# reinterpretcat/qwen3-rs

Hardware: NVIDIA B200
Metric: decode_tokens_per_s (higher is better)
Workload: dtype int8 weights x int8 activations, int32 group dots, f32 accumulate

## Files before the change

### qwen3_rs_b200/csrc/q3_engine.cu

```cuda
#include "../../include/qwen3_cuda.h"
#include "q3_kernels.cuh"
#include "q3_mega.cuh"
#include "q3_prefill.cuh"
#include "q3_sampler.cuh"
#include <cudaTypedefs.h>

#include <cuda_runtime.h>
#include <fcntl.h>
#include <math.h>
#include <stdarg.h>
#include <stdio.h>
#include <stdlib.h>
#include <string.h>
#include <sys/mman.h>
#include <sys/stat.h>
#include <unistd.h>

#include <string>
#include <vector>

using namespace q3;

static thread_local char g_err[1024] = "";
static int fail(int code, const char *fmt, ...) {
// ... 593 lines not shown
    CK(cudaFuncSetAttribute(h->mega_fn, cudaFuncAttributeMaxDynamicSharedMemorySize, (int)h->mega_smem));
    int occ = 0;
    CK(cudaOccupancyMaxActiveBlocksPerMultiprocessor(&occ, h->mega_fn, MEGA_THREADS, h->mega_smem));
    if (occ < 1) { h->mega_why = "megakernel does not fit on an SM"; return 0; }
    h->mega_ok = true;
    return 0;
}

static int launch_mega(q3_handle *h, int l0, int l1, bool from_embed, bool run_head, bool feedback, bool gather) {
    MegaArgs a = h->margs;
    a.layer0 = l0; a.layer1 = l1; a.from_embed = from_embed; a.run_head = run_head; a.feedback = feedback;
    a.gather_logits = h->tp_size > 1 ? (h->logits_root >= 0 ? (1 << h->logits_root) : (gather ? (1 << h->tp_size) - 1 : 0)) : 0;
    a.bar_base = h->bar_base;
    a.xbar_base = h->xbar_base;
    if (h->poisoned) return fail(Q3_ECOMM, "tensor-parallel handle is unusable after a timed-out wait (ranks may have diverged): destroy and re-create every rank");
    const int nbar = run_head ? 1 : 0;
    const int nx = h->tp_size > 1 ? nbar : 0;
    a.ll_base = (unsigned)(h->ll_count % 0xFFFFFFFFull);
    h->ll_count += (unsigned long long)MEGA_EDGES * (unsigned)(l1 - l0 + 1);
    void *params[] = {&a};
    CK(cudaLaunchCooperativeKernel(h->mega_fn, dim3(h->num_sms), dim3(MEGA_THREADS), params, h->mega_smem, h->stream));
    h->bar_base += (unsigned long long)(nbar - nx) * h->num_sms;
    h->xbar_base += (unsigned long long)nx * h->tp_size * h->num_sms;
    return 0;
}

static int check_tok_pos(const q3_handle *h, int token, int pos);
static int finish_call(q3_handle *h) {
    const bool mega = h->d_status && h->decode_path == 1;
    if (mega) CK(cudaMemcpyAsync(h->h_small + 16, h->d_status, 4, cudaMemcpyDeviceToHost, h->stream));
    CK(cudaStreamSynchronize(h->stream));
    if (!mega) return 0;
    const int code = h->h_small[16];
    if (code) {
        cudaMemset(h->d_status, 0, 64);
        if (h->tp_size > 1) {
            h->poisoned = true;
        } else {
            h->bar_base = 0;
            h->xbar_base = 0;
            cudaMemset(h->d_bar, 0, 64);
            cudaMemset(h->d_flags, 0, 64 * 4);
            if (h->att_cnt) cudaMemset(h->att_cnt, 0, (size_t)h->cfg.n_layers * h->n_kv_l * 4);
        }
        return fail(Q3_ECUDA, "persistent decode kernel: a wait timed out (status %d: 1 grid barrier, 2 stage ring, 3 cross-GPU barrier, 4 producer order, "
                              "6-10 flagged exchange: 6 o/down rows, 7 attention output, 8 SwiGLU outputs, 9 qkv rows, 10 TP partials; 11 prefill cross-GPU barrier)%s", code,
                    h->tp_size > 1 ? "; tensor-parallel handle poisoned" : "");
    }
    return 0;
}
extern "C" int q3_debug_profile(q3_handle *h, int token, int pos, unsigned long long *out, size_t out_words, int *n_rows_out,
                                int *n_events_out) {
    if (!h) return fail(Q3_EINVAL, "null argument");
    if (n_rows_out) *n_rows_out = 3 * h->num_sms;
    if (n_events_out) *n_events_out = MEGA_PROF_EVENTS;
    if (!out) return out_words == 0 ? Q3_OK : fail(Q3_EINVAL, "null argument");
    if (!h->mega_ok) return fail(Q3_EUNSUPPORTED, "persistent decode kernel unavailable: %s", h->mega_why.c_str());
    if (out_words < (size_t)3 * h->num_sms * MEGA_PROF_EVENTS)
        return fail(Q3_EINVAL, "profile buffer too small: %zu words, need %zu", out_words, (size_t)3 * h->num_sms * MEGA_PROF_EVENTS);
    if (int rc0 = check_tok_pos(h, token, pos)) return rc0;
    CK(cudaSetDevice(h->device));
    h->h_small[0] = token; h->h_small[1] = pos; h->h_small[2] = 0; h->h_small[3] = 0;
    CK(cudaMemcpyAsync(h->d_tokpos, h->h_small, 16, cudaMemcpyHostToDevice, h->stream));
    unsigned long long *d = nullptr;
    size_t bytes = (size_t)3 * h->num_sms * MEGA_PROF_EVENTS * 8;
    CK(cudaMalloc((void **)&d, bytes));
    CK(cudaMemsetAsync(d, 0, bytes, h->stream));
    h->margs.prof = d;
    int rc = launch_mega(h, 0, h->cfg.n_layers, true, true, false, false);
    h->margs.prof = nullptr;
    if (!rc) {
        cudaError_t e = cudaMemcpyAsync(out, d, bytes, cudaMemcpyDeviceToHost, h->stream);
        rc = e == cudaSuccess ? finish_call(h) : fail(Q3_ECUDA, "profile copy failed: %s", cudaGetErrorString(e));
    }
    cudaFree(d);
    return rc;
}
extern "C" int q3_num_sms(const q3_handle *h) { return h ? h->num_sms : 0; }
extern "C" int q3_debug_set_epoch(q3_handle *h, unsigned long long exchanges_issued) {
    if (!h) return fail(Q3_EINVAL, "null handle");
    h->ll_count = exchanges_issued;
    return Q3_OK;
}

static inline bool use_mega(const q3_handle *h) { return h->decode_path == 1 && h->mega_ok && !h->exact; }
static int tp_ready(const q3_handle *h) {
    if (h->tp_size > 1 && !h->tp_connected) return fail(Q3_ECOMM, "tensor-parallel handle used before q3_tp_connect");
    if (h->tp_size > 1 && !use_mega(h)) return fail(Q3_EUNSUPPORTED, "under tensor parallelism only the persistent fast path is available");
    return 0;
}

enum StepOut {
    STEP_LOGITS,
    STEP_ARGMAX,
    STEP_FEEDBACK,
};
static int launch_decode_step(q3_handle *h, StepOut out, bool gather = false) {
    if (use_mega(h)) return launch_mega(h, 0, h->cfg.n_layers, true, true, out == STEP_FEEDBACK, gather);
    CK(cudaGraphLaunch(out == STEP_FEEDBACK ? h->g_greedy[h->exact] : h->g_fwd[h->exact], h->stream));
    if (out == STEP_ARGMAX) launch_argmax(h, false, h->stream);
    return 0;
}
static int launch_head_only(q3_handle *h, bool gather) {
    if (use_mega(h)) return launch_mega(h, 0, 0, false, true, false, gather);
    launch_head(h, h->stream);
    return 0;
}

static PFN_cuTensorMapEncodeTiled_v12000 get_encode_fn() {
    static PFN_cuTensorMapEncodeTiled_v12000 fn = nullptr;
    if (!fn) {
        void *p = nullptr;
        cudaDriverEntryPointQueryResult qres;
        if (cudaGetDriverEntryPoint("cuTensorMapEncodeTiled", &p, cudaEnableDefault, &qres) == cudaSuccess && qres == cudaDriverEntryPointSuccess)
            fn = (PFN_cuTensorMapEncodeTiled_v12000)p;
    }
    return fn;
}
// ... 1292 lines not shown
```

### qwen3_rs_b200/csrc/q3_mega.cuh

```cuda
#pragma once
#include <cuda.h>

#include "q3_kernels.cuh"

namespace q3 {

#ifndef MEGA_GW_
#define MEGA_GW_ 8
#endif
constexpr int MEGA_GW = MEGA_GW_;
constexpr int MEGA_BATCH = 4 * MEGA_GW;
constexpr int MEGA_GROUPS = 2;
constexpr int MEGA_NCW = MEGA_GW * MEGA_GROUPS;
constexpr int MEGA_CTHREADS = MEGA_NCW * 32;
constexpr int MEGA_THREADS = MEGA_CTHREADS + 32 * MEGA_GROUPS;
#ifndef MEGA_NSTAGE_
#define MEGA_NSTAGE_ 4
#endif
constexpr int MEGA_NSTAGE = MEGA_NSTAGE_;
constexpr int MEGA_MAX_KT = 4096;
constexpr int MEGA_SCRATCH = 40960;
constexpr int MEGA_MAX_TP = 8;
constexpr int MEGA_MAX_SPLITS = ATTN_MAX_SPLITS;
constexpr int MEGA_EDGES = 6;

enum { PH_QKV = 0, PH_O = 1, PH_GU = 2, PH_DN = 3, PH_HEAD = 4 };

struct MegaGemv {
    const uint8_t *base;
    long long layer_stride;
    int units;
    int K, n_kt, KT, G;
    int tile_bytes;
};

constexpr int MEGA_KV_ROWS = 32;

struct MegaArgs {
    alignas(64) CUtensorMap map_k;
    alignas(64) CUtensorMap map_v;
    int dim, n_layers, n_heads_l, n_kv_l, AH_l, KV_l, H_l, vocab_l, vocab_row0, seq_len;
    int tp_rank, tp_size;
    MegaGemv g[5];
    const float *rms_att, *rms_ffn, *q_ln, *k_ln, *rms_final;
    const int8_t *embed_q;
    const float *embed_s;
    const float *rope;
    float *kc, *vc;
    float *x;
    unsigned long long *zq;
    unsigned long long *za;
    unsigned long long *zh;
    unsigned long long *zr[2];
    unsigned long long *part[2][MEGA_MAX_TP];
    float *attn_part;
    unsigned *att_cnt;
    float *logits[MEGA_MAX_TP];
    unsigned long long *best[MEGA_MAX_TP];
    unsigned long long *bar;
    unsigned long long bar_base;
    unsigned long long *xbar[MEGA_MAX_TP];
    unsigned long long xbar_base;
    int *tokpos, *history;
    int *status;
    int layer0, layer1, from_embed, run_head, feedback, gather_logits;
    unsigned ll_base;
    unsigned long long *prof;
};
constexpr int MEGA_PROF_EVENTS = 4096;
struct Prof {
    unsigned long long *row;
    int ev;
};
// ... 75 lines not shown
    unsigned long long x;
    asm volatile("ld.relaxed.sys.global.b64 %0, [%1];" : "=l"(x) : "l"(p) : "memory");
    return x;
}
__device__ __forceinline__ bool ll_ok(unsigned long long w, unsigned epoch) { return (unsigned)(w >> 32) == epoch; }
__device__ __noinline__ bool ll_give_up(const MegaArgs &a, unsigned &spins, int code) {
    if ((++spins & 255u) == 0) {
        if (*(volatile int *)a.status) return true;
        if (spins > (1u << 20)) {
            atomicExch(a.status, code);
            return true;
        }
    }
    return false;
}
__device__ __forceinline__ float4 ll_poll4(const MegaArgs &a, const unsigned long long *p, unsigned epoch, int code) {
    unsigned long long w0, w1, w2, w3;
    unsigned spins = 0;
    while (true) {
        ll_load2(p, w0, w1);
        ll_load2(p + 2, w2, w3);
        if (ll_ok(w0, epoch) && ll_ok(w1, epoch) && ll_ok(w2, epoch) && ll_ok(w3, epoch)) break;
        if (ll_give_up(a, spins, code)) break;
    }
    return make_float4(__uint_as_float((unsigned)w0), __uint_as_float((unsigned)w1), __uint_as_float((unsigned)w2), __uint_as_float((unsigned)w3));
}

__device__ __host__ __forceinline__ void cta_share(int units, int nctas, int c, int &start, int &count) {
    int base = units / nctas, rem = units % nctas;
    count = base + (c < rem ? 1 : 0);
    start = c * base + (c < rem ? c : rem);
}

template <int GS>
__global__ void __launch_bounds__(256) k_build_stream(const int8_t *__restrict__ src_q, const float *__restrict__ src_s,
                                                      uint8_t *dst, int units, int K, int n_kt, int nctas, int pair) {
    constexpr int CPG = GS / 16;
    const int u = blockIdx.x, kt = blockIdx.y;
    const int KT = K / n_kt, G = KT / GS, tile_bytes = KT + ((4 * G + 15) & ~15);
    const int base = units / nctas, rem = units % nctas;
    int c, j;
    if (u < rem * (base + 1)) {
        c = u / (base + 1);
        j = u % (base + 1);
    } else {
        c = rem + (u - rem * (base + 1)) / base;
        j = (u - rem * (base + 1)) % base;
    }
    int start, n_c;
    cta_share(units, nctas, c, start, n_c);
    for (int half = 0; half < (pair ? 2 : 1); half++) {
        long long tile_index;
        size_t src_row;
        if (pair) {
            int blk = j / MEGA_GW, w = j % MEGA_GW, np = n_c - MEGA_GW * blk;
            if (np > MEGA_GW) np = MEGA_GW;
            tile_index = (long long)start * 2 + 2 * MEGA_GW * blk + half * np + w;
            src_row = (size_t)2 * u + half;
        } else {
            int b = j / MEGA_BATCH, jb = j % MEGA_BATCH, nb = n_c - MEGA_BATCH * b;
            if (nb > MEGA_BATCH) nb = MEGA_BATCH;
            tile_index = ((long long)start + MEGA_BATCH * b) * n_kt + (long long)kt * nb + jb;
            src_row = (size_t)u;
        }
        uint8_t *tile = dst + tile_index * tile_bytes;
        const int8_t *srow = src_q + src_row * K + (size_t)kt * KT;
        for (int ch = threadIdx.x; ch < KT / 16; ch += blockDim.x) {
            int g = ch / CPG, p = ch % CPG, b = g / 32, l = g % 32;
            int ngb = G - 32 * b;
            if (ngb > 32) ngb = 32;
            int dpos = b * 32 * CPG + p * ngb + l;
            reinterpret_cast<int4 *>(tile)[dpos] = reinterpret_cast<const int4 *>(srow)[ch];
        }
        const float *ss = src_s + src_row * (K / GS) + (size_t)kt * G;
        for (int g = threadIdx.x; g < G; g += blockDim.x) reinterpret_cast<float *>(tile + KT)[g] = ss[g];
    }
}

__device__ __forceinline__ int4 lds128(uint32_t saddr) {
    int4 r;
    asm volatile("ld.shared.v4.b32 {%0,%1,%2,%3}, [%4];" : "=r"(r.x), "=r"(r.y), "=r"(r.z), "=r"(r.w) : "r"(saddr));
    return r;
}
__device__ __forceinline__ float lds_f32(uint32_t saddr) {
    float r;
    asm volatile("ld.shared.f32 %0, [%1];" : "=f"(r) : "r"(saddr));
    return r;
}
template <int GS>
struct XRegs {
    static constexpr int CPG = GS / 16;
    static constexpr int NBLK = MEGA_MAX_KT / (32 * GS);
    int4 x[NBLK][CPG];
    float s[NBLK];
};

template <int GS>
__device__ __forceinline__ int xq_offset(int i4, int KT, int G) {
    int r = i4 * 4, off = 0;
    while (r >= KT) {
        r -= KT;
        off += KT;
    }
    const int g = r / GS, b = g >> 5, l = g & 31;
    int ngb = G - 32 * b;
    ngb = ngb > 32 ? 32 : ngb;
    const int p = (r % GS) >> 4;
    return off + b * 32 * GS + (p * ngb + l) * 16 + (r & 15);
}
template <int GS>
__device__ __forceinline__ void xq_store(uint8_t *sxq, int i4, uint32_t packed, int KT, int G) {
    *reinterpret_cast<uint32_t *>(sxq + xq_offset<GS>(i4, KT, G)) = packed;
}
template <int GS>
__device__ __forceinline__ void load_x(XRegs<GS> &xr, const uint8_t *sxq, const float *sxs, int kt, int KT, int G, int lane) {
    const uint32_t base = smem_u32(sxq) + kt * KT + lane * 16;
#pragma unroll
    for (int b = 0; b < XRegs<GS>::NBLK; b++) {
        int ngb = G - 32 * b;
        ngb = ngb > 32 ? 32 : ngb;
        const bool ok = lane < ngb;
        if (ngb < 1) ngb = 1;
        xr.s[b] = ok ? sxs[kt * G + b * 32 + lane] : 0.0f;
#pragma unroll
        for (int p = 0; p < XRegs<GS>::CPG; p++)
            xr.x[b][p] = ok ? lds128(base + b * 32 * GS + p * ngb * 16) : make_int4(0, 0, 0, 0);
    }
}

template <int GS, bool FULL>
__device__ __forceinline__ float tile_dot(uint32_t tile, const XRegs<GS> &xr, int KT, int G, int lane) {
    constexpr int CPG = XRegs<GS>::CPG;
    constexpr int NBLK = XRegs<GS>::NBLK;
    int4 w[NBLK][CPG];
    float ws[NBLK];
#pragma unroll
    for (int b = 0; b < NBLK; b++) {
        int ngb = FULL ? 32 : (G - 32 * b > 32 ? 32 : G - 32 * b);
        const bool on = FULL ? (32 * b < G) : (lane < ngb);
        if (!FULL && ngb < 1) ngb = 1;
        const uint32_t base = tile + b * 32 * GS + lane * 16;
#pragma unroll
        for (int p = 0; p < CPG; p++) w[b][p] = on ? lds128(base + p * ngb * 16) : make_int4(0, 0, 0, 0);
        ws[b] = on ? lds_f32(tile + KT + (b * 32 + lane) * 4) : 0.0f;
    }
    float acc = 0.0f;
#pragma unroll
    for (int b = 0; b < NBLK; b++) {
        int d0 = 0, d1 = 0;
#pragma unroll
        for (int p = 0; p < CPG; p += 2) {
            d0 = dot16(w[b][p], xr.x[b][p], d0);
            d1 = dot16(w[b][p + 1], xr.x[b][p + 1], d1);
        }
        acc = __fadd_rn(acc, __fmul_rn(__fmul_rn((float)(d0 + d1), ws[b]), xr.s[b]));
    }
    return warp_sum(acc);
}

constexpr int MEGA_MAXV = (MEGA_MAX_KT + 4 * MEGA_CTHREADS - 1) / (4 * MEGA_CTHREADS);

template <int GS>
__device__ __noinline__ void prologue_norm(const MegaArgs &a, const float *w, int src, const unsigned long long *zone, unsigned epoch,
                                           uint8_t *sxq, float *sxs, float *sred, float *sx, int KT, int G, Prof &pr) {
    const int tid = threadIdx.x, lane = tid & 31, warp = tid >> 5;
    const int n4 = a.dim >> 2;
    constexpr int MAXV = MEGA_MAXV;
    float4 v[MAXV], wv[MAXV];
    float ss = 0.0f;
#pragma unroll
    for (int k = 0; k < MAXV; k++) {
        const int i4 = tid + k * MEGA_CTHREADS;
        wv[k] = (i4 < n4) ? __ldg(reinterpret_cast<const float4 *>(w) + i4) : make_float4(0.f, 0.f, 0.f, 0.f);
    }
#pragma unroll
    for (int k = 0; k < MAXV; k++) {
        const int i4 = tid + k * MEGA_CTHREADS;
        v[k] = make_float4(0.f, 0.f, 0.f, 0.f);
        if (i4 < n4) {
            if (src == 0) {
                size_t base = (size_t)a.tokpos[0] * a.dim + (size_t)i4 * 4;
                char4 e = *reinterpret_cast<const char4 *>(a.embed_q + base);
                float sc = a.embed_s[base / GS];
                v[k] = make_float4((float)e.x * sc, (float)e.y * sc, (float)e.z * sc, (float)e.w * sc);
            } else if (src == 1) {
                v[k] = ldcg_f4(a.x + (size_t)i4 * 4);
            } else {
                v[k] = reinterpret_cast<const float4 *>(sx)[i4];
            }
        }
    }
    if (zone) {
        unsigned long long ww[MAXV][4];
        unsigned spins = 0;
        while (true) {
            bool ok = true;
#pragma unroll
            for (int k = 0; k < MAXV; k++) {
                const int i4 = tid + k * MEGA_CTHREADS;
                if (i4 < n4) {
                    ll_load2(zone + (size_t)i4 * 4, ww[k][0], ww[k][1]);
                    ll_load2(zone + (size_t)i4 * 4 + 2, ww[k][2], ww[k][3]);
                    ok = ok && ll_ok(ww[k][0], epoch) && ll_ok(ww[k][1], epoch) && ll_ok(ww[k][2], epoch) && ll_ok(ww[k][3], epoch);
                }
            }
            if (ok || ll_give_up(a, spins, 6)) break;
        }
#pragma unroll
// ... 474 lines not shown
                asm volatile("ld.acquire.gpu.global.u64 %0, [%1];" : "=l"(v) : "l"(a.bar) : "memory");
                if (v >= bs.target) break;
                if ((++spins & 1023u) == 0) {
                    if (*st) break;
                    if (clock64() - t0 > 4000000000LL) {
                        atomicExch(a.status, 1);
                        break;
                    }
                }
            }
        }
    }
    if (x) bs.xtarget += (unsigned long long)a.tp_size * gridDim.x;
    else bs.target += gridDim.x;
    prof_mark(pr, 41);
    csync();
}

struct PhaseGeom {
    const uint8_t *seg;
    int start, count;
};
struct MegaShared {
    int start[5], count[5];
    long long seg_off[5], seg_len[5];
    unsigned long long *part[2][MEGA_MAX_TP];
    float *logits[MEGA_MAX_TP];
    unsigned long long *best[MEGA_MAX_TP];
};
__device__ __forceinline__ PhaseGeom phase_geom(const MegaArgs &a, const MegaShared &sh, int ph, int layer) {
    PhaseGeom pg;
    pg.start = sh.start[ph];
    pg.count = sh.count[ph];
    pg.seg = a.g[ph].base + (long long)layer * a.g[ph].layer_stride + sh.seg_off[ph];
    return pg;
}

template <int GS, int KVMUL>
__global__ void __launch_bounds__(MEGA_THREADS, 1) k_mega_decode(const __grid_constant__ MegaArgs a) {
    extern __shared__ __align__(1024) uint8_t mega_smem[];
    uint8_t *smem = mega_smem;
    const int slot_bytes = MEGA_GW * (MEGA_MAX_KT + 4 * (MEGA_MAX_KT / GS));
    uint8_t *ring = smem;
    uint8_t *scratch = smem + MEGA_NSTAGE * slot_bytes;
    uint8_t *sxq = scratch;
    float *sxs = reinterpret_cast<float *>(scratch + 16384);
    float *sred = reinterpret_cast<float *>(scratch + 16384 + 2048);
    uint64_t *full = reinterpret_cast<uint64_t *>(scratch + MEGA_SCRATCH);
    uint64_t *empty = full + MEGA_GROUPS * MEGA_NSTAGE;
    MegaShared &sh = *reinterpret_cast<MegaShared *>(scratch + MEGA_SCRATCH + 192);
    static_assert(192 + sizeof(MegaShared) <= 1024, "MegaShared outgrew its slot");
    float *sx = reinterpret_cast<float *>(scratch + MEGA_SCRATCH + 1024);
    volatile unsigned *issued = reinterpret_cast<volatile unsigned *>(scratch + MEGA_SCRATCH + 128);
    const int tid = threadIdx.x, lane = tid & 31, warp = tid >> 5;

    if (tid == 0) {
        for (int s = 0; s < MEGA_NSTAGE; s++) {
            mbar_init(&full[s], 1);
            mbar_init(&full[MEGA_NSTAGE + s], 1);
            mbar_init(&empty[s], MEGA_GW);
            issued[s] = 0;
        }
        asm volatile("fence.mbarrier_init.release.cluster;" ::: "memory");
#pragma unroll 1
        for (int ph = 0; ph < 5; ph++) {
            int st, cn;
            cta_share(a.g[ph].units, gridDim.x, blockIdx.x, st, cn);
            const long long per_unit = (long long)(ph == PH_GU ? 2 : 1) * a.g[ph].n_kt * a.g[ph].tile_bytes;
            sh.start[ph] = st;
            sh.count[ph] = cn;
            sh.seg_off[ph] = st * per_unit;
            sh.seg_len[ph] = cn * per_unit;
        }
    }
    if (tid < MEGA_MAX_TP) {
        sh.part[0][tid] = a.part[0][tid];
        sh.part[1][tid] = a.part[1][tid];
        sh.logits[tid] = a.logits[tid];
        sh.best[tid] = a.best[tid];
    }
    __syncthreads();

    const int L0 = a.layer0, L1 = a.layer1;

    if (warp >= MEGA_NCW) {
        if (lane != 0) return;
        const int pw = warp - MEGA_NCW;
        uint64_t policy;
        asm volatile("createpolicy.fractional.L2::evict_first.b64 %0, 1.0;" : "=l"(policy));
        unsigned it = 0;
        Prof pr;
        pr.row = (a.prof && pw == 0) ? a.prof + (size_t)(gridDim.x + blockIdx.x) * MEGA_PROF_EVENTS : nullptr;
        pr.ev = 0;
        auto push = [&](const uint8_t *src, int nr, int tile_bytes, int owner) {
            if (owner != pw) {
                it++;
                return;
            }
            const int slot = it % MEGA_NSTAGE;
            const uint32_t bytes = (uint32_t)nr * tile_bytes;
            {
                const unsigned use = it / MEGA_NSTAGE;
                long long t0 = clock64();
                while (issued[slot] != use) {
                    if (clock64() - t0 > 4000000000LL) { atomicExch(a.status, 4); break; }
                }
            }
            mbar_wait(&empty[slot], ((it / MEGA_NSTAGE) & 1) ^ 1, a.status);
            uint64_t *fb = &full[owner * MEGA_NSTAGE + slot];
            mbar_expect_tx(fb, bytes);
            bulk_g2s(ring + (size_t)slot * slot_bytes, src, bytes, fb, policy);
            __threadfence_block();
            issued[slot] = it / MEGA_NSTAGE + 1;
            prof_mark(pr, 64 + slot);
            it++;
        };
        const int ppos = a.tokpos[1];
        const int pns = mega_nsplit(ppos, a.n_kv_l, gridDim.x);
        const bool has_item = (int)blockIdx.x < a.n_kv_l * pns;
        const int pkvh = blockIdx.x % a.n_kv_l, psplit = blockIdx.x / a.n_kv_l;
        const int pper = (ppos + 1 + pns - 1) / pns;
        const int pt0 = psplit * pper, pt1 = pt0 + pper < ppos + 1 ? pt0 + pper : ppos + 1;
        auto kvpush = [&](int layer) {
            if (!has_item) return;
            for (int t = pt0, si = 0; t < pt1; t += MEGA_KV_ROWS, si++) {
                const int owner = si & 1;
                if (owner != pw) {
                    it++;
                    continue;
                }
                const int slot = it % MEGA_NSTAGE;
                {
                    const unsigned use = it / MEGA_NSTAGE;
                    long long tw = clock64();
                    while (issued[slot] != use) {
                        if (clock64() - tw > 4000000000LL) { atomicExch(a.status, 4); break; }
                    }
                }
                mbar_wait(&empty[slot], ((it / MEGA_NSTAGE) & 1) ^ 1, a.status);
                uint64_t *fb = &full[owner * MEGA_NSTAGE + slot];
                uint8_t *dst = ring + (size_t)slot * slot_bytes;
                mbar_expect_tx(fb, 2 * MEGA_KV_ROWS * HEAD_DIM * 4);
                tma_load_2d(dst, &a.map_k, pkvh * HEAD_DIM, layer * a.seq_len + t, fb);
                tma_load_2d(dst + MEGA_KV_ROWS * HEAD_DIM * 4, &a.map_v, pkvh * HEAD_DIM, layer * a.seq_len + t, fb);
                __threadfence_block();
                issued[slot] = it / MEGA_NSTAGE + 1;
                prof_mark(pr, 64 + slot);
                it++;
            }
        };
        auto plain = [&](int ph, int layer) {
            const MegaGemv &g = a.g[ph];
            PhaseGeom pg = phase_geom(a, sh, ph, layer);
            const uint8_t *src = pg.seg;
            for (int b0 = 0; b0 < pg.count; b0 += MEGA_BATCH) {
                int nb = pg.count - b0 < MEGA_BATCH ? pg.count - b0 : MEGA_BATCH;
                for (int kt = 0; kt < g.n_kt; kt++)
                    for (int s = 0, si = 0; s < nb; s += MEGA_GW, si++) {
                        int nr = nb - s < MEGA_GW ? nb - s : MEGA_GW;
                        push(src, nr, g.tile_bytes, si & 1);
                        src += (size_t)nr * g.tile_bytes;
                    }
            }
        };
        auto pairs = [&](int layer) {
            const MegaGemv &g = a.g[PH_GU];
            PhaseGeom pg = phase_geom(a, sh, PH_GU, layer);
            const uint8_t *src = pg.seg;
            for (int p0 = 0, bi = 0; p0 < pg.count; p0 += MEGA_GW, bi++) {
                int np = pg.count - p0 < MEGA_GW ? pg.count - p0 : MEGA_GW;
                for (int half = 0; half < 2; half++) {
                    push(src, np, g.tile_bytes, bi & 1);
                    src += (size_t)np * g.tile_bytes;
                }
            }
        };
        for (int l = L0; l < L1; l++) {
            plain(PH_QKV, l);
            kvpush(l);
            plain(PH_O, l);
            pairs(l);
            plain(PH_DN, l);
        }
        if (a.run_head) plain(PH_HEAD, 0);
        if (pr.row) pr.row[MEGA_PROF_EVENTS - 1] = (unsigned long long)pr.ev;
        return;
    }

    unsigned it = 0;
    BarState bs;
    bs.target = a.bar_base + gridDim.x;
    bs.xtarget = a.xbar_base + (unsigned long long)a.tp_size * gridDim.x;
    const int pos = a.tokpos[1];
    const int grp = warp / MEGA_GW, wl = warp % MEGA_GW;
    Prof pr;
    pr.row = (a.prof && (tid == 0 || tid == MEGA_GW * 32)) ? a.prof + (size_t)((tid ? 2 * gridDim.x : 0) + blockIdx.x) * MEGA_PROF_EVENTS : nullptr;
    pr.ev = 0;
    unsigned fullp = 0;
    uint64_t *myfull = full + grp * MEGA_NSTAGE;
    XRegs<GS> xr;
    prof_mark(pr, 0);
    long long best = (long long)0x8000000000000000LL;
    const int n_layer_steps = 5 * (L1 - L0);
    const int n_steps = n_layer_steps + (a.run_head ? 1 : 0);
    const int nsplit = mega_nsplit(pos, a.n_kv_l, gridDim.x);

    for (int step = 0; step < n_steps; step++) {
        const bool head = step >= n_layer_steps;
        const int l = head ? 0 : L0 + step / 5;
        const int kind = head ? 5 : step % 5;
        const unsigned ep_step = ll_epoch(a.ll_base, head ? (unsigned)(MEGA_EDGES * (L1 - L0)) : (unsigned)(MEGA_EDGES * (l - L0) + kind));
        const unsigned ep_prev = ll_epoch(a.ll_base, (unsigned)(MEGA_EDGES * (l - L0) + kind - 1));
        int ph = PH_QKV;
        if (kind == 0 || kind == 3 || kind == 5) {
            const float *w = kind == 0 ? a.rms_att + (size_t)l * a.dim : kind == 3 ? a.rms_ffn + (size_t)l * a.dim : a.rms_final;
            const bool emb = kind == 0 && l == L0 && a.from_embed;
            const bool pending = kind == 3 || (kind == 0 ? l > L0 : L1 > L0);
            ph = kind == 0 ? PH_QKV : kind == 3 ? PH_GU : PH_HEAD;
            const unsigned ep_rows = kind == 3 ? ep_prev : ll_epoch(a.ll_base, (unsigned)(MEGA_EDGES * ((kind == 0 ? l - 1 : L1 - 1) - L0) + 4));
            prologue_norm<GS>(a, w, emb ? 0 : (pending ? 2 : 1), pending ? a.zr[kind == 3 ? 0 : 1] : nullptr, ep_rows, sxq, sxs, sred, sx,
                              a.g[ph].KT, a.g[ph].G, pr);
        } else if (kind == 1) {
            if ((int)blockIdx.x < a.n_kv_l * nsplit) {
                RingPos rp{it, fullp};
                attention_item<GS, KVMUL>(a, l, pos, blockIdx.x % a.n_kv_l, blockIdx.x / a.n_kv_l, nsplit, scratch, ep_prev, ep_step, pr, rp,
                                          smem_u32(ring), slot_bytes, myfull, empty);
                it = rp.it;
                fullp = rp.fullp;
            }
        } else if (kind == 2) {
            prologue_attn_poll<GS>(a, ep_prev, sxq, sxs);
            ph = PH_O;
        } else {
            prologue_quant_ll<GS>(a, a.zh, ep_prev, a.H_l, sxq, sxs, a.g[PH_DN].KT, a.g[PH_DN].G);
            ph = PH_DN;
        }
        prof_mark(pr, 1 + 3 * kind);
        if (kind != 1) {
            const MegaGemv &g = a.g[ph];
            const int start = sh.start[ph], count = sh.count[ph];
            const bool full_blocks = (g.G & 31) == 0;
            const uint32_t ring_s = smem_u32(ring);
            if (kind == 3) {
                const unsigned ep_h = ep_step;
                load_x<GS>(xr, sxq, sxs, 0, g.KT, g.G, lane);
                for (int p0 = 0, bi = 0; p0 < count; p0 += MEGA_GW, bi++) {
                    const int np = count - p0 < MEGA_GW ? count - p0 : MEGA_GW;
                    if ((bi & 1) != grp) {
                        it += 2;
                        continue;
                    }
                    float gate = 0.0f, up = 0.0f;
                    for (int half = 0; half < 2; half++) {
                        const int slot = it % MEGA_NSTAGE;
                        mbar_wait(&myfull[slot], (fullp >> slot) & 1, a.status);
                        fullp ^= 1u << slot;
                        prof_mark(pr, 48 + slot);
                        {
                            const uint32_t tile = ring_s + slot * slot_bytes + wl * g.tile_bytes;
                            float v = full_blocks ? tile_dot<GS, true>(tile, xr, g.KT, g.G, lane) : tile_dot<GS, false>(tile, xr, g.KT, g.G, lane);
                            gate = half == 0 ? v : gate;
                            up = half == 0 ? up : v;
                        }
                        __syncwarp();
                        if (lane == 0) mbar_arrive(&empty[slot]);
                        it++;
                    }
                    if (wl < np && lane == 0) {
                        float sw = __fmul_rn(gate, __fdiv_rn(1.0f, __fadd_rn(1.0f, expf(-gate))));
                        ll_store(a.zh + start + p0 + wl, __fmul_rn(sw, up), ep_h);
                    }
                }
            } else {
                const unsigned ep_out = ep_step;
                for (int b0 = 0; b0 < count; b0 += MEGA_BATCH) {
                    const int nb = count - b0 < MEGA_BATCH ? count - b0 : MEGA_BATCH;
                    float acc0 = 0.f, acc1 = 0.f;
                    for (int kt = 0; kt < g.n_kt; kt++) {
                        load_x<GS>(xr, sxq, sxs, kt, g.KT, g.G, lane);
                        prof_mark(pr, 58);
                        for (int sidx = 0; MEGA_GW * sidx < nb; sidx++) {
                            if ((sidx & 1) == grp) {
                                const int slot = it % MEGA_NSTAGE;
                                mbar_wait(&myfull[slot], (fullp >> slot) & 1, a.status);
                                fullp ^= 1u << slot;
                                prof_mark(pr, 48 + slot);
                                {
                                    const uint32_t tile = ring_s + slot * slot_bytes + wl * g.tile_bytes;
                                    float v = full_blocks ? tile_dot<GS, true>(tile, xr, g.KT, g.G, lane) : tile_dot<GS, false>(tile, xr, g.KT, g.G, lane);
                                    v = (MEGA_GW * sidx + wl < nb) ? v : 0.0f;
                                    acc0 += sidx < 2 ? v : 0.0f;
                                    acc1 += sidx < 2 ? 0.0f : v;
                                    prof_mark(pr, 59);
                                }
                                __syncwarp();
                                if (lane == 0) mbar_arrive(&empty[slot]);
                            }
                            it++;
                        }
                    }
                    if (lane == 0) {
                        for (int j = 0; j < 2; j++) {
                            const int sidx = grp + 2 * j;
                            if (MEGA_GW * sidx + wl >= nb) break;
                            const int r = start + b0 + MEGA_GW * sidx + wl;
                            const float v = j == 0 ? acc0 : acc1;
                            if (kind == 0) {
                                ll_store(a.zq + r, v, ep_out);
                            } else if (kind == 2 || kind == 4) {
                                if (a.tp_size == 1) {
                                    ll_store(a.zr[kind == 2 ? 0 : 1] + r, v, ep_out);
                                } else {
                                    unsigned long long *const *dst = sh.part[kind == 2 ? 0 : 1];
#pragma unroll 1
                                    for (int p = 0; p < a.tp_size; p++) ll_store(dst[p] + (size_t)a.tp_rank * a.dim + r, v, ep_out);
                                }
                            } else {
                                const int row = a.vocab_row0 + r;
                                sh.logits[a.tp_rank][row] = v;
                                if (a.gather_logits) {
#pragma unroll 1
                                    for (int p = 0; p < a.tp_size; p++)
                                        if (p != a.tp_rank && ((a.gather_logits >> p) & 1)) sh.logits[p][row] = v;
                                }
                                long long key = ((long long)total_key(v) << 32) | (unsigned)row;
                                best = key > best ? key : best;
                            }
                        }
                    }
                }
                if ((kind == 2 || kind == 4) && a.tp_size > 1) {
                    const unsigned long long *src = sh.part[kind == 2 ? 0 : 1][a.tp_rank];
                    for (int idx = tid; idx < count; idx += MEGA_CTHREADS) {
                        const int r = start + idx;
                        unsigned long long w[MEGA_MAX_TP];
                        unsigned spins = 0;
                        while (true) {
                            bool ok = true;
#pragma unroll
                            for (int p = 0; p < MEGA_MAX_TP; p++) {
                                if (p < a.tp_size) {
                                    w[p] = ll_load1(src + (size_t)p * a.dim + r);
                                    ok = ok && ll_ok(w[p], ep_out);
                                }
                            }
                            if (ok || ll_give_up(a, spins, 10)) break;
                        }
                        float s = __uint_as_float((unsigned)w[0]);
#pragma unroll
                        for (int p = 1; p < MEGA_MAX_TP; p++)
                            if (p < a.tp_size) s = __fadd_rn(s, __uint_as_float((unsigned)w[p]));
                        ll_store(a.zr[kind == 2 ? 0 : 1] + r, s, ep_out);
                    }
                }
            }
        }
        prof_mark(pr, 2 + 3 * kind);
        if (kind == 5) {
            long long *sbest = reinterpret_cast<long long *>(sred + 32);
            if (lane == 0) sbest[warp] = best;
            csync();
            if (tid == 0) {
                for (int w = 1; w < MEGA_NCW; w++) best = sbest[w] > best ? sbest[w] : best;
#pragma unroll 1
                for (int p = 0; p < a.tp_size; p++) sh.best[p][(size_t)a.tp_rank * gridDim.x + blockIdx.x] = (unsigned long long)best;
            }
        }
        if (kind == 2 || kind == 4) {
            const float *wn = kind == 2 ? a.rms_ffn + (size_t)l * a.dim : (l + 1 < L1 ? a.rms_att + (size_t)(l + 1) * a.dim : a.rms_final);
            if (tid * 32 < a.dim) asm volatile("prefetch.global.L2 [%0];" ::"l"(wn + tid * 32));
        } else if (kind == 0 && tid < 12) {
            const float *wn = tid < 4 ? a.q_ln + (size_t)l * HEAD_DIM + tid * 32 : tid < 8 ? a.k_ln + (size_t)l * HEAD_DIM + (tid - 4) * 32
                                                                                   : a.rope + (size_t)pos * HEAD_DIM + (tid - 8) * 32;
            asm volatile("prefetch.global.L2 [%0];" ::"l"(wn));
        }
        if (kind == 5) grid_barrier(a, bs, true, pr);
        else csync();
        prof_mark(pr, 3 + 3 * kind);
    }

    if (pr.row) pr.row[MEGA_PROF_EVENTS - 1] = (unsigned long long)pr.ev;
    if (a.run_head) {
        if (blockIdx.x == 0 && warp == 0) {
            long long b = (long long)0x8000000000000000LL;
            const int n = a.tp_size * gridDim.x;
            for (int i = lane; i < n; i += 32) {
                long long k = (long long)__ldcg(sh.best[a.tp_rank] + i);
                b = k > b ? k : b;
            }
#pragma unroll
            for (int o = 16; o > 0; o >>= 1) {
                long long other = __shfl_xor_sync(0xffffffffu, b, o);
                b = other > b ? other : b;
            }
            if (lane == 0) {
                int tok = (int)(b & 0xffffffffLL);
                a.tokpos[2] = tok;
                if (a.feedback) {
                    a.tokpos[0] = tok;
                    a.tokpos[1] = pos + 1;
                    a.history[a.tokpos[3]] = tok;
                    a.tokpos[3] += 1;
                }
            }
        }
    } else if (blockIdx.x == 0 && L1 > L0) {
        const unsigned ep = ll_epoch(a.ll_base, (unsigned)(MEGA_EDGES * (L1 - 1 - L0) + 4));
        for (int i4 = tid; i4 < (a.dim >> 2); i4 += MEGA_CTHREADS) {
            float4 v = reinterpret_cast<const float4 *>(sx)[i4];
            const float4 d = ll_poll4(a, a.zr[1] + (size_t)i4 * 4, ep, 6);
            v.x = __fadd_rn(v.x, d.x);
            v.y = __fadd_rn(v.y, d.y);
            v.z = __fadd_rn(v.z, d.z);
            v.w = __fadd_rn(v.w, d.w);
            reinterpret_cast<float4 *>(a.x)[i4] = v;
        }
    }
}

}
```

Baseline: 449.5.

## Stage weight tiles through tensor memory via a dedicated tcgen05 copier warp

Adds a copier warp that allocates tensor memory and moves full 8-row weight tiles from the shared-memory ring into a TMEM ring with tcgen05.cp. Compute warps then read the weights and scales with tcgen05.ld instead of shared-memory loads. Weights are repacked offline into a 128-lane layout that matches the TMEM copy shape. The intent is to release shared-memory stage slots sooner and cut shared-memory load pressure in the GEMV dot products. The cost is an extra warp, extra barriers and handoff latency, plus sensitivity to getting the TMEM descriptors right.

Measured after the change: 453.1, median of 6. About the same (+0.8%).

```diff
diff --git a/qwen3_rs_b200/csrc/q3_engine.cu b/qwen3_rs_b200/csrc/q3_engine.cu
--- a/qwen3_rs_b200/csrc/q3_engine.cu
+++ b/qwen3_rs_b200/csrc/q3_engine.cu
@@ -669,18 +669,18 @@
 extern "C" int q3_debug_profile(q3_handle *h, int token, int pos, unsigned long long *out, size_t out_words, int *n_rows_out,
                                 int *n_events_out) {
     if (!h) return fail(Q3_EINVAL, "null argument");
-    if (n_rows_out) *n_rows_out = 3 * h->num_sms;
+    if (n_rows_out) *n_rows_out = 4 * h->num_sms;
     if (n_events_out) *n_events_out = MEGA_PROF_EVENTS;
     if (!out) return out_words == 0 ? Q3_OK : fail(Q3_EINVAL, "null argument");
     if (!h->mega_ok) return fail(Q3_EUNSUPPORTED, "persistent decode kernel unavailable: %s", h->mega_why.c_str());
-    if (out_words < (size_t)3 * h->num_sms * MEGA_PROF_EVENTS)
-        return fail(Q3_EINVAL, "profile buffer too small: %zu words, need %zu", out_words, (size_t)3 * h->num_sms * MEGA_PROF_EVENTS);
+    if (out_words < (size_t)4 * h->num_sms * MEGA_PROF_EVENTS)
+        return fail(Q3_EINVAL, "profile buffer too small: %zu words, need %zu", out_words, (size_t)4 * h->num_sms * MEGA_PROF_EVENTS);
     if (int rc0 = check_tok_pos(h, token, pos)) return rc0;
     CK(cudaSetDevice(h->device));
     h->h_small[0] = token; h->h_small[1] = pos; h->h_small[2] = 0; h->h_small[3] = 0;
     CK(cudaMemcpyAsync(h->d_tokpos, h->h_small, 16, cudaMemcpyHostToDevice, h->stream));
     unsigned long long *d = nullptr;
-    size_t bytes = (size_t)3 * h->num_sms * MEGA_PROF_EVENTS * 8;
+    size_t bytes = (size_t)4 * h->num_sms * MEGA_PROF_EVENTS * 8;
     CK(cudaMalloc((void **)&d, bytes));
     CK(cudaMemsetAsync(d, 0, bytes, h->stream));
     h->margs.prof = d;
diff --git a/qwen3_rs_b200/csrc/q3_mega.cuh b/qwen3_rs_b200/csrc/q3_mega.cuh
--- a/qwen3_rs_b200/csrc/q3_mega.cuh
+++ b/qwen3_rs_b200/csrc/q3_mega.cuh
@@ -13,12 +13,27 @@
 constexpr int MEGA_GROUPS = 2;
 constexpr int MEGA_NCW = MEGA_GW * MEGA_GROUPS;
 constexpr int MEGA_CTHREADS = MEGA_NCW * 32;
-constexpr int MEGA_THREADS = MEGA_CTHREADS + 32 * MEGA_GROUPS;
+constexpr int MEGA_COPIER = MEGA_NCW + MEGA_GROUPS;
+constexpr int MEGA_THREADS = MEGA_CTHREADS + 32 * (MEGA_GROUPS + 1);
 #ifndef MEGA_NSTAGE_
 #define MEGA_NSTAGE_ 4
 #endif
 constexpr int MEGA_NSTAGE = MEGA_NSTAGE_;
 constexpr int MEGA_MAX_KT = 4096;
+constexpr int MEGA_TM_SCOL = 2 * (MEGA_MAX_KT / 128);
+template <int GS>
+struct TmRing {
+    static constexpr int NBLK = MEGA_MAX_KT / (32 * GS);
+    static constexpr int COLS = MEGA_TM_SCOL + 2 * NBLK;
+#ifdef MEGA_TDEPTH_
+    static constexpr int DEPTH = MEGA_TDEPTH_;
+#else
+    static constexpr int DEPTH = 512 / COLS;
+#endif
+    static_assert(DEPTH >= 2 && DEPTH <= 8 && DEPTH * COLS <= 512, "tensor-memory ring depth");
+    static_assert(MEGA_GW == 8, "two row tiles per lane quadrant");
+};
+__device__ __host__ __forceinline__ bool tm_stage(int G, int nr) { return G % 64 == 0 && nr == MEGA_GW; }
 constexpr int MEGA_SCRATCH = 40960;
 constexpr int MEGA_MAX_TP = 8;
 constexpr int MEGA_MAX_SPLITS = ATTN_MAX_SPLITS;
@@ -200,19 +215,38 @@
     for (int half = 0; half < (pair ? 2 : 1); half++) {
         long long tile_index;
         size_t src_row;
+        int wl, nr;
         if (pair) {
             int blk = j / MEGA_GW, w = j % MEGA_GW, np = n_c - MEGA_GW * blk;
             if (np > MEGA_GW) np = MEGA_GW;
             tile_index = (long long)start * 2 + 2 * MEGA_GW * blk + half * np + w;
             src_row = (size_t)2 * u + half;
+            wl = w;
+            nr = np;
         } else {
             int b = j / MEGA_BATCH, jb = j % MEGA_BATCH, nb = n_c - MEGA_BATCH * b;
             if (nb > MEGA_BATCH) nb = MEGA_BATCH;
             tile_index = ((long long)start + MEGA_BATCH * b) * n_kt + (long long)kt * nb + jb;
             src_row = (size_t)u;
+            wl = jb % MEGA_GW;
+            nr = nb - (jb - wl) < MEGA_GW ? nb - (jb - wl) : MEGA_GW;
+        }
+        const int8_t *srow = src_q + src_row * K + (size_t)kt * KT;
+        const float *ss = src_s + src_row * (K / GS) + (size_t)kt * G;
+        if (tm_stage(G, nr)) {
+            uint8_t *stage = dst + (tile_index - wl) * tile_bytes;
+            const int CH = KT / 512, NB = G / 32, h = wl >> 2, r0 = (wl & 3) * 32;
+            for (int ch = threadIdx.x; ch < KT / 16; ch += blockDim.x) {
+                int g = ch / CPG, p = ch % CPG, b = g / 32, l = g % 32;
+                reinterpret_cast<int4 *>(stage + (size_t)(h * CH + b * CPG + p) * 2048)[r0 + l] = reinterpret_cast<const int4 *>(srow)[ch];
+            }
+            for (int g = threadIdx.x; g < G; g += blockDim.x) {
+                const int w = h * NB + g / 32;
+                reinterpret_cast<float *>(stage + (size_t)(2 * CH + w / 4) * 2048)[(r0 + g % 32) * 4 + w % 4] = ss[g];
+            }
+            continue;
         }
         uint8_t *tile = dst + tile_index * tile_bytes;
-        const int8_t *srow = src_q + src_row * K + (size_t)kt * KT;
         for (int ch = threadIdx.x; ch < KT / 16; ch += blockDim.x) {
             int g = ch / CPG, p = ch % CPG, b = g / 32, l = g % 32;
             int ngb = G - 32 * b;
@@ -220,7 +254,6 @@
             int dpos = b * 32 * CPG + p * ngb + l;
             reinterpret_cast<int4 *>(tile)[dpos] = reinterpret_cast<const int4 *>(srow)[ch];
         }
-        const float *ss = src_s + src_row * (K / GS) + (size_t)kt * G;
         for (int g = threadIdx.x; g < G; g += blockDim.x) reinterpret_cast<float *>(tile + KT)[g] = ss[g];
     }
 }
@@ -302,6 +335,76 @@
             d1 = dot16(w[b][p + 1], xr.x[b][p + 1], d1);
         }
         acc = __fadd_rn(acc, __fmul_rn(__fmul_rn((float)(d0 + d1), ws[b]), xr.s[b]));
+    }
+    return warp_sum(acc);
+}
+
+__device__ __forceinline__ void tm_fence_after() { asm volatile("tcgen05.fence::after_thread_sync;" ::: "memory"); }
+__device__ __forceinline__ void tm_fence_before() { asm volatile("tcgen05.fence::before_thread_sync;" ::: "memory"); }
+__device__ __forceinline__ bool elect_one() {
+    uint32_t pred;
+    asm volatile("{\n.reg .pred p;\nelect.sync _|p, 0xffffffff;\nselp.u32 %0, 1, 0, p;\n}" : "=r"(pred));
+    return pred != 0;
+}
+__device__ __forceinline__ void tm_cp(uint32_t taddr, uint32_t saddr) {
+    const uint64_t desc = (uint64_t)((saddr & 0x3FFFF) >> 4) | ((uint64_t)(128 >> 4) << 16) | ((uint64_t)(128 >> 4) << 32) | (1ULL << 46);
+    asm volatile("tcgen05.cp.cta_group::1.128x128b [%0], %1;" ::"r"(taddr), "l"(desc) : "memory");
+}
+__device__ __forceinline__ void tm_commit(uint64_t *bar) {
+    asm volatile("tcgen05.commit.cta_group::1.mbarrier::arrive::one.shared::cluster.b64 [%0];" ::"r"(smem_u32(bar)) : "memory");
+}
+__device__ __forceinline__ void mbar_arrive_n(uint64_t *bar, uint32_t n) {
+    asm volatile("mbarrier.arrive.shared::cta.b64 _, [%0], %1;" ::"r"(smem_u32(bar)), "r"(n) : "memory");
+}
+template <int N>
+__device__ __forceinline__ void tm_ld(uint32_t (&r)[N], uint32_t taddr) {
+    static_assert(N == 1 || N == 2 || N == 4 || N == 32, "tcgen05.ld shape");
+    if constexpr (N == 32) {
+        asm volatile("tcgen05.ld.sync.aligned.32x32b.x32.b32 {%0,%1,%2,%3,%4,%5,%6,%7,%8,%9,%10,%11,%12,%13,%14,%15,%16,%17,%18,%19,%20,%21,%22,"
+                     "%23,%24,%25,%26,%27,%28,%29,%30,%31}, [%32];"
+                     : "=r"(r[0]), "=r"(r[1]), "=r"(r[2]), "=r"(r[3]), "=r"(r[4]), "=r"(r[5]), "=r"(r[6]), "=r"(r[7]), "=r"(r[8]), "=r"(r[9]),
+                       "=r"(r[10]), "=r"(r[11]), "=r"(r[12]), "=r"(r[13]), "=r"(r[14]), "=r"(r[15]), "=r"(r[16]), "=r"(r[17]), "=r"(r[18]),
+                       "=r"(r[19]), "=r"(r[20]), "=r"(r[21]), "=r"(r[22]), "=r"(r[23]), "=r"(r[24]), "=r"(r[25]), "=r"(r[26]), "=r"(r[27]),
+                       "=r"(r[28]), "=r"(r[29]), "=r"(r[30]), "=r"(r[31])
+                     : "r"(taddr)
+                     : "memory");
+    } else if constexpr (N == 4) {
+        asm volatile("tcgen05.ld.sync.aligned.32x32b.x4.b32 {%0,%1,%2,%3}, [%4];" : "=r"(r[0]), "=r"(r[1]), "=r"(r[2]), "=r"(r[3]) : "r"(taddr) : "memory");
+    } else if constexpr (N == 2) {
+        asm volatile("tcgen05.ld.sync.aligned.32x32b.x2.b32 {%0,%1}, [%2];" : "=r"(r[0]), "=r"(r[1]) : "r"(taddr) : "memory");
+    } else {
+        asm volatile("tcgen05.ld.sync.aligned.32x32b.x1.b32 {%0}, [%1];" : "=r"(r[0]) : "r"(taddr) : "memory");
+    }
+}
+
+template <int GS>
+__device__ __forceinline__ float tile_dot_tm(uint32_t tcol, uint32_t scol, uint64_t *tempty, const XRegs<GS> &xr, int G, int lane) {
+    constexpr int CPG = XRegs<GS>::CPG;
+    constexpr int NBLK = XRegs<GS>::NBLK;
+    uint32_t r[32], sc[NBLK];
+    __syncwarp();
+    tm_fence_after();
+    tm_ld(r, tcol);
+    tm_ld(sc, scol);
+    asm volatile("tcgen05.wait::ld.sync.aligned;" ::: "memory");
+    tm_fence_before();
+    __syncwarp();
+    if (lane == 0) mbar_arrive(tempty);
+    float acc = 0.0f;
+#pragma unroll
+    for (int b = 0; b < NBLK; b++) {
+        const bool on = 32 * b < G;
+        int d0 = 0, d1 = 0;
+#pragma unroll
+        for (int p = 0; p < CPG; p += 2) {
+            const int c = 4 * (b * CPG + p);
+            const int4 w0 = on ? make_int4(r[c], r[c + 1], r[c + 2], r[c + 3]) : make_int4(0, 0, 0, 0);
+            const int4 w1 = on ? make_int4(r[c + 4], r[c + 5], r[c + 6], r[c + 7]) : make_int4(0, 0, 0, 0);
+            d0 = dot16(w0, xr.x[b][p], d0);
+            d1 = dot16(w1, xr.x[b][p + 1], d1);
+        }
+        const float ws = on ? __uint_as_float(sc[b]) : 0.0f;
+        acc = __fadd_rn(acc, __fmul_rn(__fmul_rn((float)(d0 + d1), ws), xr.s[b]));
     }
     return warp_sum(acc);
 }
@@ -882,6 +985,13 @@
     static_assert(192 + sizeof(MegaShared) <= 1024, "MegaShared outgrew its slot");
     float *sx = reinterpret_cast<float *>(scratch + MEGA_SCRATCH + 1024);
     volatile unsigned *issued = reinterpret_cast<volatile unsigned *>(scratch + MEGA_SCRATCH + 128);
+    constexpr int TD = TmRing<GS>::DEPTH;
+    uint64_t *cfull = reinterpret_cast<uint64_t *>(scratch + MEGA_SCRATCH + 640);
+    uint64_t *tfull = cfull + MEGA_NSTAGE;
+    uint64_t *tempty = tfull + MEGA_GROUPS * TD;
+    uint64_t *tdone = tempty + TD;
+    uint32_t *tm_base_s = reinterpret_cast<uint32_t *>(tdone + 1);
+    static_assert(192 + sizeof(MegaShared) <= 640 && 640 + 8 * (MEGA_NSTAGE + 3 * 8 + 1) + 4 <= 1024, "barrier area");
     const int tid = threadIdx.x, lane = tid & 31, warp = tid >> 5;
 
     if (tid == 0) {
@@ -889,8 +999,15 @@
             mbar_init(&full[s], 1);
             mbar_init(&full[MEGA_NSTAGE + s], 1);
             mbar_init(&empty[s], MEGA_GW);
+            mbar_init(&cfull[s], 1);
             issued[s] = 0;
         }
+        for (int s = 0; s < TD; s++) {
+            mbar_init(&tfull[s], 1);
+            mbar_init(&tfull[TD + s], 1);
+            mbar_init(&tempty[s], MEGA_GW);
+        }
+        mbar_init(tdone, 1);
         asm volatile("fence.mbarrier_init.release.cluster;" ::: "memory");
 #pragma unroll 1
         for (int ph = 0; ph < 5; ph++) {
@@ -909,26 +1026,61 @@
         sh.logits[tid] = a.logits[tid];
         sh.best[tid] = a.best[tid];
     }
+    if (warp == MEGA_COPIER) {
+        asm volatile("tcgen05.alloc.cta_group::1.sync.aligned.shared::cta.b32 [%0], %1;" ::"r"(smem_u32(tm_base_s)), "n"(512) : "memory");
+        asm volatile("tcgen05.relinquish_alloc_permit.cta_group::1.sync.aligned;" ::: "memory");
+    }
+    tm_fence_before();
     __syncthreads();
+    tm_fence_after();
+    const uint32_t tm_base = *tm_base_s;
 
     const int L0 = a.layer0, L1 = a.layer1;
 
     if (warp >= MEGA_NCW) {
-        if (lane != 0) return;
+        const bool copier = warp == MEGA_COPIER;
+        if (!copier && lane != 0) return;
         const int pw = warp - MEGA_NCW;
         uint64_t policy;
         asm volatile("createpolicy.fractional.L2::evict_first.b64 %0, 1.0;" : "=l"(policy));
         unsigned it = 0;
         Prof pr;
-        pr.row = (a.prof && pw == 0) ? a.prof + (size_t)(gridDim.x + blockIdx.x) * MEGA_PROF_EVENTS : nullptr;
+        pr.row = (a.prof && (pw == 0 || copier)) ? a.prof + (size_t)((copier ? 3 : 1) * gridDim.x + blockIdx.x) * MEGA_PROF_EVENTS : nullptr;
         pr.ev = 0;
-        auto push = [&](const uint8_t *src, int nr, int tile_bytes, int owner) {
+        unsigned tk = 0, cfp = 0;
+        const uint32_t ring_s = smem_u32(ring);
+        auto push = [&](const uint8_t *src, int nr, const MegaGemv &g, int owner) {
+            const bool tm = tm_stage(g.G, nr);
+            if (copier) {
+                if (tm) {
+                    const int slot = it % MEGA_NSTAGE, ts = tk % TD;
+                    mbar_wait(&cfull[slot], (cfp >> slot) & 1, a.status);
+                    cfp ^= 1u << slot;
+                    mbar_wait(&tempty[ts], ((tk / TD) & 1) ^ 1, a.status);
+                    __syncwarp();
+                    tm_fence_after();
+                    if (elect_one()) {
+                        mbar_arrive_n(&empty[slot], MEGA_GW - 1);
+                        const uint32_t sb = ring_s + slot * slot_bytes, tb = tm_base + ts * TmRing<GS>::COLS;
+                        const int CH = g.KT / 512;
+                        for (int j = 0; j < 2 * CH; j++) tm_cp(tb + (j / CH) * (MEGA_TM_SCOL / 2) + (j % CH) * 4, sb + j * 2048);
+                        for (int k = 0; k < g.G / 64; k++) tm_cp(tb + MEGA_TM_SCOL + 4 * k, sb + (2 * CH + k) * 2048);
+                        tm_commit(&empty[slot]);
+                        tm_commit(&tfull[owner * TD + ts]);
+                    }
+                    __syncwarp();
+                    if (lane == 0) prof_mark(pr, 72 + ts);
+                    tk++;
+                }
+                it++;
+                return;
+            }
             if (owner != pw) {
                 it++;
                 return;
             }
             const int slot = it % MEGA_NSTAGE;
-            const uint32_t bytes = (uint32_t)nr * tile_bytes;
+            const uint32_t bytes = (uint32_t)nr * g.tile_bytes;
             {
                 const unsigned use = it / MEGA_NSTAGE;
                 long long t0 = clock64();
@@ -937,7 +1089,7 @@
                 }
             }
             mbar_wait(&empty[slot], ((it / MEGA_NSTAGE) & 1) ^ 1, a.status);
-            uint64_t *fb = &full[owner * MEGA_NSTAGE + slot];
+            uint64_t *fb = tm ? &cfull[slot] : &full[owner * MEGA_NSTAGE + slot];
             mbar_expect_tx(fb, bytes);
             bulk_g2s(ring + (size_t)slot * slot_bytes, src, bytes, fb, policy);
             __threadfence_block();
@@ -953,6 +1105,10 @@
         const int pt0 = psplit * pper, pt1 = pt0 + pper < ppos + 1 ? pt0 + pper : ppos + 1;
         auto kvpush = [&](int layer) {
             if (!has_item) return;
+            if (copier) {
+                it += (pt1 - pt0 + MEGA_KV_ROWS - 1) / MEGA_KV_ROWS;
+                return;
+            }
             for (int t = pt0, si = 0; t < pt1; t += MEGA_KV_ROWS, si++) {
                 const int owner = si & 1;
                 if (owner != pw) {
@@ -988,7 +1144,7 @@
                 for (int kt = 0; kt < g.n_kt; kt++)
                     for (int s = 0, si = 0; s < nb; s += MEGA_GW, si++) {
                         int nr = nb - s < MEGA_GW ? nb - s : MEGA_GW;
-                        push(src, nr, g.tile_bytes, si & 1);
+                        push(src, nr, g, si & 1);
                         src += (size_t)nr * g.tile_bytes;
                     }
             }
@@ -1000,7 +1156,7 @@
             for (int p0 = 0, bi = 0; p0 < pg.count; p0 += MEGA_GW, bi++) {
                 int np = pg.count - p0 < MEGA_GW ? pg.count - p0 : MEGA_GW;
                 for (int half = 0; half < 2; half++) {
-                    push(src, np, g.tile_bytes, bi & 1);
+                    push(src, np, g, bi & 1);
                     src += (size_t)np * g.tile_bytes;
                 }
             }
@@ -1013,7 +1169,18 @@
             plain(PH_DN, l);
         }
         if (a.run_head) plain(PH_HEAD, 0);
-        if (pr.row) pr.row[MEGA_PROF_EVENTS - 1] = (unsigned long long)pr.ev;
+        if (pr.row && lane == 0) pr.row[MEGA_PROF_EVENTS - 1] = (unsigned long long)pr.ev;
+        if (copier) {
+            if (elect_one()) tm_commit(tdone);
+            __syncwarp();
+            while (!mbar_try_wait(tdone, 0)) {
+            }
+            __syncwarp();
+            tm_fence_before();
+            asm volatile("bar.sync 4, %0;" ::"n"(MEGA_CTHREADS + 32) : "memory");
+            tm_fence_after();
+            asm volatile("tcgen05.dealloc.cta_group::1.sync.aligned.b32 %0, %1;" ::"r"(tm_base), "n"(512) : "memory");
+        }
         return;
     }
 
@@ -1028,7 +1195,18 @@
     pr.ev = 0;
     unsigned fullp = 0;
     uint64_t *myfull = full + grp * MEGA_NSTAGE;
+    unsigned tk = 0, tfp = 0;
+    uint64_t *mytfull = tfull + grp * TD;
     XRegs<GS> xr;
+    const uint32_t tm_q = tm_base + ((uint32_t)((wl & 3) * 32) << 16);
+    auto dot_tm = [&](const MegaGemv &g, int slot) {
+        const int ts = tk % TD;
+        mbar_wait(&mytfull[ts], (tfp >> ts) & 1, a.status);
+        tfp ^= 1u << ts;
+        prof_mark(pr, 48 + slot);
+        const uint32_t t = tm_q + ts * TmRing<GS>::COLS;
+        return tile_dot_tm<GS>(t + (wl >> 2) * (MEGA_TM_SCOL / 2), t + MEGA_TM_SCOL + (wl >> 2) * (g.G / 32), &tempty[ts], xr, g.G, lane);
+    };
     prof_mark(pr, 0);
     long long best = (long long)0x8000000000000000LL;
     const int n_layer_steps = 5 * (L1 - L0);
@@ -1076,24 +1254,30 @@
                 load_x<GS>(xr, sxq, sxs, 0, g.KT, g.G, lane);
                 for (int p0 = 0, bi = 0; p0 < count; p0 += MEGA_GW, bi++) {
                     const int np = count - p0 < MEGA_GW ? count - p0 : MEGA_GW;
+                    const bool tm = tm_stage(g.G, np);
                     if ((bi & 1) != grp) {
                         it += 2;
+                        tk += tm ? 2 : 0;
                         continue;
                     }
                     float gate = 0.0f, up = 0.0f;
                     for (int half = 0; half < 2; half++) {
                         const int slot = it % MEGA_NSTAGE;
-                        mbar_wait(&myfull[slot], (fullp >> slot) & 1, a.status);
-                        fullp ^= 1u << slot;
-                        prof_mark(pr, 48 + slot);
-                        {
+                        float v;
+                        if (tm) {
+                            v = dot_tm(g, slot);
+                            tk++;
+                        } else {
+                            mbar_wait(&myfull[slot], (fullp >> slot) & 1, a.status);
+                            fullp ^= 1u << slot;
+                            prof_mark(pr, 48 + slot);
                             const uint32_t tile = ring_s + slot * slot_bytes + wl * g.tile_bytes;
-                            float v = full_blocks ? tile_dot<GS, true>(tile, xr, g.KT, g.G, lane) : tile_dot<GS, false>(tile, xr, g.KT, g.G, lane);
-                            gate = half == 0 ? v : gate;
-                            up = half == 0 ? up : v;
+                            v = full_blocks ? tile_dot<GS, true>(tile, xr, g.KT, g.G, lane) : tile_dot<GS, false>(tile, xr, g.KT, g.G, lane);
+                            __syncwarp();
+                            if (lane == 0) mbar_arrive(&empty[slot]);
                         }
-                        __syncwarp();
-                        if (lane == 0) mbar_arrive(&empty[slot]);
+                        gate = half == 0 ? v : gate;
+                        up = half == 0 ? up : v;
                         it++;
                     }
                     if (wl < np && lane == 0) {
@@ -1110,22 +1294,27 @@
                         load_x<GS>(xr, sxq, sxs, kt, g.KT, g.G, lane);
                         prof_mark(pr, 58);
                         for (int sidx = 0; MEGA_GW * sidx < nb; sidx++) {
+                            const bool tm = tm_stage(g.G, nb - MEGA_GW * sidx < MEGA_GW ? nb - MEGA_GW * sidx : MEGA_GW);
                             if ((sidx & 1) == grp) {
                                 const int slot = it % MEGA_NSTAGE;
-                                mbar_wait(&myfull[slot], (fullp >> slot) & 1, a.status);
-                                fullp ^= 1u << slot;
-                                prof_mark(pr, 48 + slot);
-                                {
+                                float v;
+                                if (tm) {
+                                    v = dot_tm(g, slot);
+                                } else {
+                                    mbar_wait(&myfull[slot], (fullp >> slot) & 1, a.status);
+                                    fullp ^= 1u << slot;
+                                    prof_mark(pr, 48 + slot);
                                     const uint32_t tile = ring_s + slot * slot_bytes + wl * g.tile_bytes;
-                                    float v = full_blocks ? tile_dot<GS, true>(tile, xr, g.KT, g.G, lane) : tile_dot<GS, false>(tile, xr, g.KT, g.G, lane);
-                                    v = (MEGA_GW * sidx + wl < nb) ? v : 0.0f;
-                                    acc0 += sidx < 2 ? v : 0.0f;
-                                    acc1 += sidx < 2 ? 0.0f : v;
-                                    prof_mark(pr, 59);
+                                    v = full_blocks ? tile_dot<GS, true>(tile, xr, g.KT, g.G, lane) : tile_dot<GS, false>(tile, xr, g.KT, g.G, lane);
+                                    __syncwarp();
+                                    if (lane == 0) mbar_arrive(&empty[slot]);
                                 }
-                                __syncwarp();
-                                if (lane == 0) mbar_arrive(&empty[slot]);
+                                v = (MEGA_GW * sidx + wl < nb) ? v : 0.0f;
+                                acc0 += sidx < 2 ? v : 0.0f;
+                                acc1 += sidx < 2 ? 0.0f : v;
+                                prof_mark(pr, 59);
                             }
+                            tk += tm ? 1 : 0;
                             it++;
                         }
                     }
@@ -1210,6 +1399,8 @@
     }
 
     if (pr.row) pr.row[MEGA_PROF_EVENTS - 1] = (unsigned long long)pr.ev;
+    tm_fence_before();
+    asm volatile("bar.sync 4, %0;" ::"n"(MEGA_CTHREADS + 32) : "memory");
     if (a.run_head) {
         if (blockIdx.x == 0 && warp == 0) {
             long long b = (long long)0x8000000000000000LL;
```
